# Furyton/Recommender-Baseline-Model

Hardware: AMD Instinct MI355X
Metric: training sequences/sec, SASRec L=200 d=128 at 1/2/4/8 MI355X; HR@10 parity (higher is better)
Workload: dtype bf16; 1 GPU; SASRec ML-1M shape (|items|=3416, seq_len=200, d=128, 2 blocks, 1 head, dropout 0.2); model=SASRec, global_batch=128, per_gpu_batch=128, seq_len=200, hidden=128, blocks=2, heads=1, num_items=3416, parallelism=dp1, hip_graph=True, bench_config=cfg2, sampler=host, steps_per_graph=10, full=False

## Files before the change

include/recsys_hip.h:

```cpp
#ifndef RECSYS_HIP_H
#define RECSYS_HIP_H
#include <stdint.h>
#ifdef __cplusplus
extern "C" {
#endif

#define RS_ERR_ARG 1001
#define RS_ERR_UNSUPPORTED 1002

typedef struct rs_epilogue {
  const float* bias;
  float alpha;
  int act;
  const void* aux;
  void* aux_out;
  int64_t ldaux;
  float drop_p;
  uint64_t drop_seed;
  const uint64_t* seed_base;
  int64_t drop_ld;
  const void* resid;
  int64_t ldres;
  const int64_t* rowmask_ids;
  int accumulate;
// ... 183 lines not shown
                          const float* divisor, void* f, float* pl, float* nl, float* dpl, float* dnl, void* dx,
                          float* lnpart, float* part, void* stream);

int64_t rs_touched_rows_ws_numel(int64_t rows);
int rs_touched_rows(const int64_t* ids, int64_t n, int64_t rows, int32_t* flags, int32_t* index, int32_t* count,
                    int32_t* ws, void* stream);
int rs_rows_pack(const float* src, int64_t rows, int64_t d, const int32_t* index, const int32_t* count,
                 float* compact, int64_t cap, void* stream);
int rs_rows_unpack(float* dst, int64_t rows, int64_t d, const int32_t* index, const float* compact, void* stream);

int64_t rs_sas_block_parts(int64_t M);
int rs_sas_block_out_bwd(int64_t M, int64_t d, const void* dxn, const int64_t* ids, const void* h1, const void* x1,
                         const float* mean2, const float* rstd2, const float* ln_w, const void* W2T, const void* W1T,
                         const void* WoT, void* dy2, void* da1, void* dx1, void* dout, float* part, float drop_p,
                         uint64_t salt1, uint64_t salt2, const uint64_t* seed_base, void* stream);
int rs_sas_block_out_bwd_delta(int64_t M, int64_t d, const void* dxn, const int64_t* ids, const void* h1,
                               const void* x1, const float* mean2, const float* rstd2, const float* ln_w,
                               const void* W2T, const void* W1T, const void* WoT, void* dy2, void* da1, void* dx1,
                               void* dout, float* part, float drop_p, uint64_t salt1, uint64_t salt2,
                               const uint64_t* seed_base, const void* o, float* delta, void* stream);
int rs_sas_block_in_bwd(int64_t M, int64_t d, const void* dq, const void* dkv, const void* dx1, const void* x,
                        const float* mean1, const float* rstd1, const float* ln_w, const void* WinT, void* dx,
                        float* part, void* stream);
int rs_transpose_bf16(int64_t nmat, const int64_t* desc, int64_t max_tiles, const void* src, void* dst,
                      void* stream);

typedef struct {
  const void* dY; int64_t lddy;
  const void* X;  int64_t ldx;
  int64_t N, K;
  float* dW;
  float* db;
} rs_wgrad_problem;
typedef struct {
  const float* src; int64_t stride; int64_t splits; int64_t n; float* out;
} rs_reduce_segment;
int64_t rs_wgrad_grouped_slab_numel(int nprob, const rs_wgrad_problem* probs, int64_t M, int64_t rows_per_split);
int rs_wgrad_grouped_tile(int nprob, const rs_wgrad_problem* probs);
int rs_wgrad_grouped_tile_max(int nprob, const rs_wgrad_problem* probs, int max_tile);
int rs_wgrad_grouped(int nprob, const rs_wgrad_problem* probs, int64_t M, int64_t rows_per_split, float* slab,
                     int64_t slab_numel, int nextra, const rs_reduce_segment* extra, void* stream);
int rs_wgrad_grouped_max(int nprob, const rs_wgrad_problem* probs, int64_t M, int64_t rows_per_split, float* slab,
                         int64_t slab_numel, int nextra, const rs_reduce_segment* extra, int max_tile, void* stream);

int rs_wgrad_grouped_pos(int nprob, const rs_wgrad_problem* probs, int64_t M, int64_t rows_per_split, float* slab,
                         int64_t slab_numel, int nextra, const rs_reduce_segment* extra, const int64_t* ids,
// ... 75 lines not shown
```

recommender-baseline-model_amd/_lib.py:

```python
import ctypes as C
import os

import torch

PKG = os.path.dirname(os.path.abspath(__file__))
LIB_PATH = os.path.join(PKG, "librecsys_hip.so" if not os.environ.get("RS_LIB_VARIANT")
                        else f"librecsys_hip.{os.environ['RS_LIB_VARIANT']}.so")

F32, BF16 = 0, 1

i32, i64, u64, f32, f64, vp = C.c_int, C.c_int64, C.c_uint64, C.c_float, C.c_double, C.c_void_p


class Epilogue(C.Structure):
    _fields_ = [
        ("bias", vp), ("alpha", f32), ("act", i32),
        ("aux", vp), ("aux_out", vp), ("ldaux", i64),
        ("drop_p", f32), ("drop_seed", u64), ("seed_base", vp), ("drop_ld", i64),
        ("resid", vp), ("ldres", i64),
        ("rowmask_ids", vp), ("accumulate", i32),
        ("post_drop_p", f32), ("post_drop_seed", u64), ("rows_dev", vp),
    ]


# ... 59 lines not shown
    "rs_vocab_shard_lse": [i64, i64, i64, vp, i64, vp, i64, vp, vp, vp, vp, vp],
    "rs_vocab_shard_label_logits": [i64, i64, vp, i64, vp, i64, vp, vp, i64, i64, vp, vp],
    "rs_vocab_shard_combine": [i32, i64, vp, vp, vp, vp, vp, vp],
    "rs_seed_advance": [vp, vp],
    "rs_sas_block_parts": [i64],
    "rs_touched_rows_ws_numel": [i64],
    "rs_touched_rows": [vp, i64, i64, vp, vp, vp, vp, vp],
    "rs_rows_pack": [vp, i64, i64, vp, vp, vp, i64, vp],
    "rs_rows_unpack": [vp, i64, i64, vp, vp, vp],
    "rs_sas_block_in": [i64, i64, vp, i64, vp, vp, f32, vp, vp, vp, vp, vp, vp, vp, vp, vp, vp],
    "rs_sas_block_in_count_parts": [i64],
    "rs_sas_block_grid": [i64],
    "rs_sas_block_out_head": [i64, i64, vp, vp, vp, vp, vp, vp, vp, f32, vp, vp, vp, vp, vp, vp, vp, vp, vp, vp, f32,
                              u64, u64, vp, vp, vp, vp, vp, vp, vp, i64, vp, vp, vp, vp, vp, vp, vp, vp, vp, vp],
    "rs_sas_block_in_embed": [i64, i64, vp, i64, vp, vp, f32, f32, u64, vp, vp, vp, vp, vp, vp, f32, vp, vp, vp, vp,
                              vp, vp, vp, vp, vp, vp],
    "rs_sas_block_out": [i64, i64, vp, vp, vp, vp, vp, vp, vp, f32, vp, vp, vp, vp, vp, vp, vp, vp, vp, vp, f32,
                         u64, u64, vp, vp],
    "rs_sas_block_out_bwd": [i64, i64, vp, vp, vp, vp, vp, vp, vp, vp, vp, vp, vp, vp, vp, vp, vp, f32, u64, u64,
                             vp, vp],
    "rs_sas_block_out_bwd_delta": [i64, i64, vp, vp, vp, vp, vp, vp, vp, vp, vp, vp, vp, vp, vp, vp, vp, f32, u64,
                                   u64, vp, vp, vp, vp],
    "rs_sas_block_in_bwd": [i64, i64, vp, vp, vp, vp, vp, vp, vp, vp, vp, vp, vp],
    "rs_wgrad_grouped": [i32, C.POINTER(WgradProblem), i64, i64, vp, i64, i32, C.POINTER(ReduceSegment), vp],
    "rs_reduce_segments": [i32, C.POINTER(ReduceSegment), i32, vp],
    "rs_wgrad_grouped_slab_numel": [i32, C.POINTER(WgradProblem), i64, i64],
    "rs_wgrad_grouped_tile": [i32, C.POINTER(WgradProblem)],
    "rs_wgrad_grouped_tile_max": [i32, C.POINTER(WgradProblem), i32],
    "rs_wgrad_grouped_max": [i32, C.POINTER(WgradProblem), i64, i64, vp, i64, i32, C.POINTER(ReduceSegment), i32, vp],
    "rs_item_index_ws_bytes": [i32, i64, i64, i64],
    "rs_item_index_build": [i32, vp, vp, vp, i64, i64, i64, vp, i64, vp],
    "rs_item_index_layout": [i32, i64, i64, i64, C.POINTER(i64)],
    "rs_sas_head_fwd": [i64, i64, vp, vp, vp, f32, vp, vp, vp, vp, vp, vp, vp, vp, vp, vp],
    "rs_sas_head_finish": [i64, vp, vp, vp, vp],
    "rs_sas_head_bwd": [i64, i64, vp, vp, vp, vp, vp, vp, vp, vp, vp, vp, vp, vp, vp, vp, vp, vp, vp, vp, vp],
    "rs_item_grad": [vp, i32, i64, i64, i64, vp, f32, f32, u64, vp, vp, vp, vp, vp, vp],
    "rs_item_grad_marked": [vp, i32, i64, i64, i64, vp, f32, f32, u64, vp, vp, vp, vp, vp, vp, vp, vp],
    "rs_item_grad_f32": [vp, i32, i64, i64, i64, vp, f32, f32, u64, vp, vp, vp, vp, vp, vp],
    "rs_wgrad_grouped_pos": [i32, C.POINTER(WgradProblem), i64, i64, vp, i64, i32, C.POINTER(ReduceSegment),
                             vp, i64, vp, i64, f32, u64, vp, vp, vp],
    "rs_wgrad_grouped_pos_stats": [i32, C.POINTER(WgradProblem), i64, i64, vp, i64, i32, C.POINTER(ReduceSegment),
                                   vp, i64, vp, i64, f32, u64, vp, vp, vp, i64, vp, vp, vp, vp],
    "rs_transpose_bf16": [i64, vp, i64, vp, vp, vp],
    "rs_sas_sample": [vp, vp, i64, i64, i64, i64, vp, u64, vp, vp, vp, vp],
    "rs_bert_mask": [vp, vp, i64, i64, i64, i64, f64, vp, vp, u64, vp, vp, vp],
    "rs_sas_sample_draws": [vp, vp, i64, i64, i64, i64, vp, u64, vp, vp, vp, vp, vp],
# ... 57 lines not shown
```

recommender-baseline-model_amd/csrc/rowchain.hip:

```cpp
#include "common.h"
#include "../../include/recsys_hip.h"

namespace rc {

#ifdef RC_PROF
__device__ unsigned long long g_rc_prof[4096 * 8 * 16];
#define RCPROF(slot)                                                                                 \
  do {                                                                                               \
    if ((threadIdx.x & 63) == 0) g_rc_prof[(blockIdx.x * 8 + (threadIdx.x >> 6)) * 16 + (slot)] = wall_clock64(); \
  } while (0)
#else
#define RCPROF(slot) \
  do {               \
  } while (0)
#endif

#ifndef RC_HEAD_PREFETCH
#define RC_HEAD_PREFETCH 1
#endif

#ifndef RC_NOSTORE
#define RC_NOSTORE 0
#endif

// ... 135 lines not shown
  float* rw = red + wave * 2 * D;
  float sg = 0.f, sgu = 0.f;
#pragma unroll
  for (int j = 0; j < Lay<D>::J; ++j) {
    const f32x4 w = vec4<D>(gw, j, g);
#pragma unroll
    for (int e = 0; e < 4; ++e) {
      const float gy = valid ? dy.v[j][e] : 0.f;
      const float u = (float)xr.v[j >> 1][4 * (j & 1) + e] - mu;
      const float gq = gy * w[e];
      const float pg = row16_sum(gy * (u * a)), pb = row16_sum(gy);
      if (cl == 0) {
        rw[feat(j, g, e)] += pg;
        rw[D + feat(j, g, e)] += pb;
      }
      sg += gq;
      sgu += gq * u;
      dy.v[j][e] = gq;
    }
  }
  sg = row_sum(sg);
  sgu = row_sum(sgu);
  const float mg = sg / (float)D, coef = a * a * a * sgu / (float)D;
#pragma unroll
  for (int j = 0; j < Lay<D>::J; ++j)
#pragma unroll
    for (int e = 0; e < 4; ++e)
      dy.v[j][e] = a * (dy.v[j][e] - mg) - coef * ((float)xr.v[j >> 1][4 * (j & 1) + e] - mu);
}

__device__ __forceinline__ void ln_zero(float* red, int D, int lane, int wave) {
  for (int i = lane; i < 2 * D; i += 64) red[wave * 2 * D + i] = 0.f;
}
template <int D>
__device__ __forceinline__ void ln_partials(const float* red, float* part, int tid) {
  __syncthreads();
  if (tid < 2 * D) {
    const int which = tid / D, c = tid % D;
    float s = 0.f;
#pragma unroll
    for (int w = 0; w < NW; ++w) s += red[(w * 2 + which) * D + c];
    part[((int64_t)blockIdx.x * 2 + which) * D + c] = s;
  }
}

__device__ __forceinline__ int64_t n_tiles(int64_t M) { return (M + TR - 1) / TR; }
// ... 104 lines not shown
  ln_fwd<D>(acc, lv + D, lv + 2 * D, o.eps, g, mu, rs);
  round_act<D>(acc, zr);
  if (!RC_NOSTORE) store_raw<D>(o.z, D, T.m, T.ok, zr, g);
  if (T.ok && g == 0) {
    o.mean[T.m] = mu;
    o.rstd[T.m] = rs;
  }
  zero<D>(acc);
  mm<D>(w1, zr, acc, lane);
  const bool drop = o.drop_p > 0.f;
#pragma unroll
  for (int j = 0; j < Lay<D>::J; ++j) {
    float dm[4] = {1.f, 1.f, 1.f, 1.f};
    if (drop) drop4(o.drop_p, o.s1, T.m, D, j, g, dm);
    const f32x4 bb = vec4<D>(lv + 3 * D, j, g);
#pragma unroll
    for (int e = 0; e < 4; ++e) acc.v[j][e] = fmaxf(acc.v[j][e] + bb[e], 0.f) * dm[e];
  }
  round_act<D>(acc, hr);
  if (!RC_NOSTORE) store_raw<D>(o.h1, D, T.m, T.ok, hr, g);
}
template <int D>
__device__ __forceinline__ void fwd_out_b(const Raw<D>& hr, const Raw<D>& zr, const Tile& T, const bf16* w2,
                                          const float* lv, const OutFwd& o, Raw<D>& xr, int lane) {
  const int g = lane >> 4;
  const bool keep = T.ok && o.ids[T.mc] != 0;
  Act<D> acc;
  zero<D>(acc);
  mm<D>(w2, hr, acc, lane);
  const bool drop = o.drop_p > 0.f;
#pragma unroll
  for (int j = 0; j < Lay<D>::J; ++j) {
    float dm[4] = {1.f, 1.f, 1.f, 1.f};
    if (drop) drop4(o.drop_p, o.s2, T.m, D, j, g, dm);
    const f32x4 bb = vec4<D>(lv + 4 * D, j, g);
#pragma unroll
    for (int e = 0; e < 4; ++e) {
      const float v = __builtin_fmaf(acc.v[j][e] + bb[e], dm[e], (float)zr.v[j >> 1][4 * (j & 1) + e]);
      acc.v[j][e] = keep ? v : 0.f;
    }
  }
  round_act<D>(acc, xr);
  store_raw<D>(o.xn, D, T.m, T.ok, xr, g);
}

template <int D>
__device__ __forceinline__ void bwd_in_a(const Raw<D>& kr, const Raw<D>& vr, const bf16* wk, const bf16* wv,
                                         Raw<D>& dxkv, int lane) {
  Act<D> acc;
  zero<D>(acc);
  mm<D>(wk, kr, acc, lane);
  mm<D>(wv, vr, acc, lane);
  round_act<D>(acc, dxkv);
}
template <int D>
__device__ __forceinline__ void bwd_in_b(const Raw<D>& qr, const Raw<D>& rr, const Raw<D>& xr, const Raw<D>& dxkv,
                                         const Tile& T, float mu, float rs, const bf16* wq, const float* lnw,
                                         float* red, Raw<D>& dxr, int lane, int wave) {
  const int g = lane >> 4;
  Act<D> dQ;
  Raw<D> r;
  to_act<D>(dQ, rr);
  mm<D>(wq, qr, dQ, lane);
  round_act<D>(dQ, r);
  ln_bwd<D>(dQ, xr, T.ok, lnw, mu, rs, red, lane, wave);
#pragma unroll
  for (int j = 0; j < Lay<D>::J; ++j)
#pragma unroll
    for (int e = 0; e < 4; ++e) dQ.v[j][e] += (float)dxkv.v[j >> 1][4 * (j & 1) + e];
  round_act<D>(dQ, dxr);
}

struct OutBwd {
  bf16 *dy2, *da1, *dx1, *dout;
  float* delta;
  const int64_t* ids;
  float drop_p;
  uint32_t s1, s2;
};
template <int D>
__device__ __forceinline__ void bwd_out_a(const Raw<D>& dr, const Raw<D>& hr, const Tile& T, const bf16* w2,
                                          const OutBwd& o, Raw<D>& dzr, Raw<D>& dar, int lane) {
  const int g = lane >> 4;
  const bool keep = T.ok && o.ids[T.mc] != 0;
  const bool drop = o.drop_p > 0.f;
  Act<D> acc;
  Raw<D> r;
#pragma unroll
  for (int j = 0; j < Lay<D>::J; ++j) {
    float dm[4] = {1.f, 1.f, 1.f, 1.f};
    if (drop) drop4(o.drop_p, o.s2, T.m, D, j, g, dm);
#pragma unroll
    for (int e = 0; e < 4; ++e) {
      const bf16 v = keep ? dr.v[j >> 1][4 * (j & 1) + e] : (bf16)0.f;
      dzr.v[j >> 1][4 * (j & 1) + e] = v;
      acc.v[j][e] = (float)v * dm[e];
    }
  }
  round_act<D>(acc, r);
  store_raw<D>(o.dy2, D, T.m, T.ok, r, g);
  zero<D>(acc);
  mm<D>(w2, r, acc, lane);
#pragma unroll
  for (int j = 0; j < Lay<D>::J; ++j) {
    float dm[4] = {1.f, 1.f, 1.f, 1.f};
    if (drop) drop4(o.drop_p, o.s1, T.m, D, j, g, dm);
#pragma unroll
    for (int e = 0; e < 4; ++e) acc.v[j][e] = ((float)hr.v[j >> 1][4 * (j & 1) + e] > 0.f ? acc.v[j][e] : 0.f) * dm[e];
  }
  round_act<D>(acc, dar);
  store_raw<D>(o.da1, D, T.m, T.ok, dar, g);
}
template <int D>
__device__ __forceinline__ void bwd_out_b(const Raw<D>& dar, const Raw<D>& xr, const Raw<D>& dzr, const Raw<D>& orr,
                                          const Tile& T, float mu, float rs, const bf16* w1, const bf16* wo,
                                          const float* lnw, const OutBwd& o, float* red, int lane, int wave) {
  const int g = lane >> 4;
  Raw<D> r;
  Act<D> dz;
  to_act<D>(dz, dzr);
  mm<D>(w1, dar, dz, lane);
  round_act<D>(dz, r);
  ln_bwd<D>(dz, xr, T.ok, lnw, mu, rs, red, lane, wave);
  round_act<D>(dz, r);
  store_raw<D>(o.dx1, D, T.m, T.ok, r, g);
  Act<D> acc;
  zero<D>(acc);
  mm<D>(wo, r, acc, lane);
  round_act<D>(acc, r);
  store_raw<D>(o.dout, D, T.m, T.ok, r, g);
  if (o.delta) {
    float dl = 0.f;
#pragma unroll
    for (int s = 0; s < Lay<D>::S; ++s)
// ... 367 lines not shown
  };
  if (t < tr.end) load_tile(tile_of(t, a.M, cl).mc);
  {
    const bf16* const W[3] = {a.WinT + D, a.WinT + 2 * D, a.WinT};
    const int64_t ldw[3] = {a.ldwt, a.ldwt, a.ldwt};
    stage_w<D, 3>(smem, W, ldw, wave, lane);
    const float* const V[1] = {a.ln_w};
    stage_v<D, 1>(reinterpret_cast<float*>(smem + L::W), V, tid);
  }
  ln_zero(red, D, lane, wave);
  __syncthreads();
  for (; t < tr.end; t += tr.step) {
    asm volatile("" ::: "memory");
    const Tile T = tile_of(t, a.M, cl);
    if (t != tr.first) load_tile(T.mc);
    Raw<D> dxkv, dxr;
    bwd_in_a<D>(kr, vr, wslot(smem, 0, WB), wslot(smem, 1, WB), dxkv, lane);
    bwd_in_b<D>(qr, rr, xr, dxkv, T, mu, rs, wslot(smem, 2, WB), lv, red, dxr, lane, wave);
    store_raw<D>(a.dx, D, T.m, T.ok, dxr, g);
  }
  ln_partials<D>(red, a.part, tid);
}

static int g_ncu = 0;
static int64_t grid_for(int64_t M) {
  if (g_ncu == 0) {
    int dev = 0, n = 0;
    if (hipGetDevice(&dev) == hipSuccess && hipDeviceGetAttribute(&n, hipDeviceAttributeMultiprocessorCount, dev) ==
                                                 hipSuccess && n > 0)
      g_ncu = n;
    else
      g_ncu = 256;
  }
  const int64_t nt = (M + TR - 1) / TR;
  return nt < g_ncu ? nt : g_ncu;
}
template <int D> static size_t lds_fwd() { return Smem<D, 3, 5, 0>::BYTES; }
template <int D, bool HEAD> static size_t lds_out() {
  return HEAD ? Smem<D, 3, 7, 1>::BYTES : Smem<D, 3, 5, 0>::BYTES;
}
template <int D> static size_t lds_bwd() { return Smem<D, 3, 1, 1>::BYTES; }

template <typename K>
static void set_lds(K kern, size_t bytes) {
  (void)hipFuncSetAttribute(reinterpret_cast<const void*>(kern), hipFuncAttributeMaxDynamicSharedMemorySize, (int)bytes);
}
template <int D, bool HEAD>
static void launch_out_t(const OutArgs& a, hipStream_t s) {
  constexpr auto k = block_out_kernel<D, HEAD>;
  const size_t lds = lds_out<D, HEAD>();
  set_lds(k, lds);
  hipLaunchKernelGGL(k, dim3((unsigned)grid_for(a.M)), dim3(NT), lds, s, a);
}
static int launch_out(const OutArgs& a, int64_t d, void* stream) {
  hipStream_t s = (hipStream_t)stream;
  const bool head = a.h.E != nullptr;
  if (d == 64) head ? launch_out_t<64, true>(a, s) : launch_out_t<64, false>(a, s);
  else if (d == 128) head ? launch_out_t<128, true>(a, s) : launch_out_t<128, false>(a, s);
  else return RS_ERR_UNSUPPORTED;
  return (int)hipGetLastError();
}

__global__ __launch_bounds__(256) void transpose_bf16_kernel(const int64_t* __restrict__ desc, const __bf16* src,
                                                             __bf16* dst) {
  __shared__ __bf16 t[64][66];
  const int64_t* dsc = desc + 6 * blockIdx.y;
  const int64_t rows = dsc[0], cols = dsc[1];
  const int64_t tc = cdiv(cols, 64);
  const int64_t tr = blockIdx.x / tc, tcc = blockIdx.x % tc;
  if (tr * 64 >= rows) return;
  const __bf16* sp = src + dsc[2];
  __bf16* dp = dst + dsc[4];
  const int64_t lds = dsc[3], ldd = dsc[5];
  for (int e = threadIdx.x; e < 64 * 64; e += 256) {
    const int r = e / 64, c = e % 64;
    const int64_t gr = tr * 64 + r, gc = tcc * 64 + c;
    t[r][c] = (gr < rows && gc < cols) ? sp[gr * lds + gc] : (__bf16)0.f;
  }
  __syncthreads();
  for (int e = threadIdx.x; e < 64 * 64; e += 256) {
    const int c = e / 64, r = e % 64;
    const int64_t gr = tr * 64 + r, gc = tcc * 64 + c;
    if (gr < rows && gc < cols) dp[gc * ldd + gr] = t[r][c];
// ... 119 lines not shown
  return (int)hipGetLastError();
}

int rs_sas_block_in_bwd(int64_t M, int64_t d, const void* dq, const void* dkv, const void* dx1, const void* x,
                        const float* mean1, const float* rstd1, const float* ln_w, const void* WinT, void* dx,
                        float* part, void* stream) {
  if (M <= 0) return RS_ERR_ARG;
  rc::InBwdArgs a = {M, (const __bf16*)dq, (const __bf16*)dkv, (const __bf16*)dx1, (const __bf16*)x, mean1, rstd1,
                     ln_w, (const __bf16*)WinT, 3 * d, (__bf16*)dx, part};
  const dim3 grid((unsigned)rc::grid_for(M));
  hipStream_t s = (hipStream_t)stream;
  if (d == 64) {
    rc::set_lds(rc::block_in_bwd_kernel<64>, rc::lds_bwd<64>());
    hipLaunchKernelGGL(rc::block_in_bwd_kernel<64>, grid, dim3(rc::NT), rc::lds_bwd<64>(), s, a);
  } else if (d == 128) {
    rc::set_lds(rc::block_in_bwd_kernel<128>, rc::lds_bwd<128>());
    hipLaunchKernelGGL(rc::block_in_bwd_kernel<128>, grid, dim3(rc::NT), rc::lds_bwd<128>(), s, a);
  } else {
    return RS_ERR_UNSUPPORTED;
  }
  return (int)hipGetLastError();
}

int rs_transpose_bf16(int64_t nmat, const int64_t* desc, int64_t max_tiles, const void* src, void* dst,
                      void* stream) {
  if (nmat <= 0 || max_tiles <= 0) return RS_ERR_ARG;
  hipLaunchKernelGGL(rc::transpose_bf16_kernel, dim3((unsigned)max_tiles, (unsigned)nmat), dim3(256), 0,
                     (hipStream_t)stream, desc, (const __bf16*)src, (__bf16*)dst);
  return (int)hipGetLastError();
}

}
```

recommender-baseline-model_amd/models/sas_model/sas.py:

```python
import math
import os

import torch
import torch.nn as nn

from ... import ops
from ...engine_util import Workspace, as_ids, capture_event, compute_dtype, require_cuda, site_salt
from ...flat import FlatParams

LN_EPS = 1e-8
SAS_LOSSES = ("bce", "ce")


class PointWiseFeedForward(nn.Module):

    def __init__(self, hidden_units, dropout_rate):
        super().__init__()
        self.conv1 = nn.Conv1d(hidden_units, hidden_units, kernel_size=1)
        self.conv2 = nn.Conv1d(hidden_units, hidden_units, kernel_size=1)
        self.dropout_rate = dropout_rate


class SAS(nn.Module):
    def __init__(self, args):
# ... 124 lines not shown
        grads = [eng.flat.view(n, grad) for n in eng.flat.names]
        return (None, None, None, None, *grads)


class SASEngine:

    def __init__(self, model: SAS, flat: FlatParams):
        self.m = model
        self.flat = flat
        self.d = model.hidden
        self.L = model.num_blocks
        self.H = model.heads
        self.Dh = self.d // self.H
        self.p = float(model.dropout_rate)
        self.dt = model.cdtype
        self.dev = flat.device
        if self.dt == torch.bfloat16:
            flat.enable_bf16()
        self.ws = Workspace(self.dev)
        self.seed_base = torch.zeros(1, dtype=torch.int64, device=self.dev)
        self.external_seed = False
        self.adam_transposes = False
        self._wT = None
        salt0 = int(torch.randint(0, 2 ** 62, (1,)).item())
        self.salt = {"emb": site_salt(salt0, 0)}
        for i in range(self.L):
            self.salt[f"attn{i}"] = site_salt(salt0, 1 + 4 * i)
            self.salt[f"ffn1_{i}"] = site_salt(salt0, 2 + 4 * i)
            self.salt[f"ffn2_{i}"] = site_salt(salt0, 3 + 4 * i)

    def sync_compute_weights(self):
        f = self.flat
        if f.bf16 is not None:
            if not f.stale:
                ops.cast_bf16(f.data, f.bf16)
            else:
                a = 0
                for lo, hi in sorted(f.stale) + [(f.numel, f.numel)]:
                    if lo > a:
                        ops.cast_bf16(f.data[a:lo], f.bf16[a:lo])
                    a = max(a, hi)
            if self._wT is not None:
                self._refresh_transposed()

    def transposed_spec(self):
        if not self.adam_transposes or self._wT is None:
# ... 125 lines not shown
            return (self.Wf(f"attention_layernorms.{i}.weight"), self.Wf(f"attention_layernorms.{i}.bias"),
                    b["Q"], b["mu1"], b["r1"], Win[:d], bin_[:d], b["q"], Win[d:], bin_[d:], b["kv"])

        def out_args(i):
            pre, fw, b = f"attention_layers.{i}.", f"forward_layers.{i}.", lay[i]
            return (b["o"], b["Q"], self.W(pre + "out_proj.weight"), self.Wf(pre + "out_proj.bias"), b["x1"],
                    self.Wf(f"forward_layernorms.{i}.weight"), self.Wf(f"forward_layernorms.{i}.bias"), LN_EPS,
                    b["z"], b["mu2"], b["r2"], self.W(fw + "conv1.weight"), self.Wf(fw + "conv1.bias"), b["h1"],
                    self.W(fw + "conv2.weight"), self.Wf(fw + "conv2.bias"), b["xn"], ids, p,
                    self.salt[f"ffn1_{i}"], self.salt[f"ffn2_{i}"], sb)

        ln_w, ln_b, Q, mu1, r1, Wq, bq, q, Wkv, bkv, kv = in_args(0)
        if emb is not None:
            ops.sas_block_in_embed(*emb, ln_w, ln_b, LN_EPS, Q, mu1, r1, Wq, bq, q, Wkv, bkv, kv)
        else:
            ops.sas_block_in(x, ln_w, ln_b, LN_EPS, Q, mu1, r1, Wq, bq, q, Wkv, bkv, kv)
        if after_first is not None:
            after_first()
        xs = [x]
        for i in range(L):
            b = lay[i]
            ops.attn_fwd(B, T, H, Dh, b["q"], b["kv"][:, :d], b["kv"][:, d:], b["o"], b["lse"], 1.0 / math.sqrt(Dh),
                         0, ids, p, self.salt[f"attn{i}"], sb)
            if head is not None and i == L - 1:
                ops.sas_block_out_head(out_args(i), *head)
            else:
                ops.sas_block_out(*out_args(i))
            if i + 1 < L:
                ln_w, ln_b, Q, mu1, r1, Wq, bq, q, Wkv, bkv, kv = in_args(i + 1)
                ops.sas_block_in(b["xn"], ln_w, ln_b, LN_EPS, Q, mu1, r1, Wq, bq, q, Wkv, bkv, kv)
            xs.append(b["xn"])
        for i in range(L):
            b = lay[i]
            for k_ in ("Q", "mu1", "r1", "q", "kv", "o", "lse", "x1", "z", "mu2", "r2", "h1"):
                s[k_].append(b[k_])
            s["x"].append(xs[i])
        return xs[L]

    @property
    def fused_head(self):
        return ops.sas_block_fused_ok(self.d, self.dt)

    def backward(self, s, dpl, dnl, grad, loss_out=None, divisor=None, split=None, aux_out=None):
        B, T, p, ids = s["B"], s["T"], s["p"], s["ids"]
        M, d, H, Dh, L = B * T, self.d, self.H, self.Dh, self.L
        sb = s["sb"]
        e = self._buf
        G = lambda n: self.flat.view(n, grad)
        slab = self.ws.get("slab", (ops.wgrad_slab_numel(M, 2 * d, d),), torch.float32)
        wln = self.ws.get("ln", (2 * 512 * d,), torch.float32)
        wat = self.ws.get("attn", (B * H * T,), torch.float32)

        fused = ops.sas_block_fused_ok(d, self.dt)
# ... 265 lines not shown
        wat = self.ws.get("attn", (B * H * T,), torch.float32)
        probs, segs = [], list(extra_segs)
        g = [dict(dy2=e("dy2", (M, d)), da1=e("da1", (M, d)), dx1=e("dx1", (M, d)), do=e("do", (M, d)),
                  dq=e("dq", (M, d)), dkv=e("dkv", (M, 2 * d))) for _ in range(L)]

        dl = [self.ws.get(f"attn_delta{i}", (B * H * T,), torch.float32) for i in range(L)] if H == 1 else None

        def out_bwd_args(i):
            return (ids, s["h1"][i], s["x1"][i], s["mu2"][i], s["r2"][i], self.Wf(f"forward_layernorms.{i}.weight"),
                    wT[i, 5], wT[i, 4], wT[i, 3], g[i]["dy2"], g[i]["da1"], g[i]["dx1"], g[i]["do"], lnp[i, 0], p,
                    self.salt[f"ffn1_{i}"], self.salt[f"ffn2_{i}"], sb, s["o"][i] if dl else None, dl[i] if dl else None)

        def in_bwd_args(i):
            return (g[i]["dq"], g[i]["dkv"], g[i]["dx1"], s["x"][i], s["mu1"][i], s["r1"][i],
                    self.Wf(f"attention_layernorms.{i}.weight"), wT[i, 0:3].reshape(d, 3 * d))

        ops.sas_block_out_bwd(dx, *out_bwd_args(L - 1))
        for i in reversed(range(L)):
            pre, fw = f"attention_layers.{i}.", f"forward_layers.{i}."
            dq, dkv, kv = g[i]["dq"], g[i]["dkv"], s["kv"][i]
            ops.attn_bwd(B, T, H, Dh, s["q"][i], kv[:, :d], kv[:, d:], s["o"][i], g[i]["do"], s["lse"][i], dq,
                         dkv[:, :d], dkv[:, d:], 1.0 / math.sqrt(Dh), 0, ids, p, self.salt[f"attn{i}"], sb,
                         dl[i] if dl else wat, delta_in=bool(dl))
            dxi = e("dxi", (M, d))
            ops.sas_block_in_bwd(*in_bwd_args(i), dxi, lnp[i, 1])
            if i > 0:
                ops.sas_block_out_bwd(dxi, *out_bwd_args(i - 1))
            dx = dxi
            Gin, Gb = G(pre + "in_proj_weight"), G(pre + "in_proj_bias")
            probs += [(g[i]["dy2"], s["h1"][i], G(fw + "conv2.weight"), G(fw + "conv2.bias")),
                      (g[i]["da1"], s["z"][i], G(fw + "conv1.weight"), G(fw + "conv1.bias")),
                      (g[i]["dx1"], s["o"][i], G(pre + "out_proj.weight"), G(pre + "out_proj.bias")),
                      (dq, s["Q"][i], Gin[:d], Gb[:d]),
                      (dkv, s["x"][i], Gin[d:], Gb[d:])]
            segs += ops.ln_partial_segments(lnp[i, 0], M, d, G(f"forward_layernorms.{i}.weight"),
                                            G(f"forward_layernorms.{i}.bias"))
            segs += ops.ln_partial_segments(lnp[i, 1], M, d, G(f"attention_layernorms.{i}.weight"),
                                            G(f"attention_layernorms.{i}.bias"))
        rows = self._wgrad_rows(M, 6 * L)
        wslab = self.ws.get("wslab", (ops.wgrad_grouped_slab_numel([(d, d)] * 4 * L + [(2 * d, d)] * L, M, rows),),
                            torch.float32)
        join, fork = None, None
        if tail is not None:
            fork = capture_event()
            fork.record(torch.cuda.current_stream())
        ops.wgrad_grouped(probs, M, rows, wslab, extra=segs, pos=pos(dx) if pos is not None else None)
        if tail is not None:
            self._side.wait_event(fork)
            with torch.cuda.stream(self._side):
                tail(dx)
# ... 30 lines not shown
```

recommender-baseline-model_amd/ops.py:

```python
import ctypes as C
import os

import torch

from . import _lib
from ._lib import BF16, F32, Epilogue, call, ptr, stream

ACT_NONE, ACT_RELU, ACT_GELU, ACT_RELU_BWD, ACT_GELU_BWD = (
    _lib.ACT_NONE, _lib.ACT_RELU, _lib.ACT_GELU, _lib.ACT_RELU_BWD, _lib.ACT_GELU_BWD)


STAMP_KINDS = {1: "attn_bwd", 2: "wgrad_grouped", 3: "vocab_ce_fwd"}


def kernel_stamps(buf, step, kinds=()):
    mask = sum(1 << k for k, n in STAMP_KINDS.items() if n in kinds)
    call("rs_kernel_stamps", ptr(buf), ptr(step), mask)


def read_kernel_stamps(buf, khz):
    import numpy as np
    h = buf.cpu().numpy().view(np.uint64)
    steps, marks, W = int(h[1]), int(h[2]), int(h[3])
    rec = h[4:4 + steps * marks * (1 + W)].reshape(steps, marks, 1 + W)
# ... 471 lines not shown

def sas_block_out(o, Q, Wo, bo, x1, ln_w, ln_b, eps, z, mean, rstd, W1, b1, h1, W2, b2, xn, ids, drop_p,
                  salt1, salt2, seed_base):
    M, d = o.shape
    call("rs_sas_block_out", M, d, ptr(o), ptr(Q), ptr(Wo), ptr(bo), ptr(x1), ptr(ln_w), ptr(ln_b), eps, ptr(z),
         ptr(mean), ptr(rstd), ptr(W1), ptr(b1), ptr(h1), ptr(W2), ptr(b2), ptr(xn), ptr(ids), drop_p, salt1,
         salt2, ptr(seed_base), stream())


def sas_block_out_bwd(dxn, ids, h1, x1, mean2, rstd2, ln_w, W2T, W1T, WoT, dy2, da1, dx1, dout, part, drop_p, salt1,
                      salt2, seed_base, o=None, delta=None):
    M, d = dxn.shape
    call("rs_sas_block_out_bwd_delta", M, d, ptr(dxn), ptr(ids), ptr(h1), ptr(x1), ptr(mean2), ptr(rstd2),
         ptr(ln_w), ptr(W2T), ptr(W1T), ptr(WoT), ptr(dy2), ptr(da1), ptr(dx1), ptr(dout), ptr(part), drop_p, salt1,
         salt2, ptr(seed_base), ptr(o), ptr(delta), stream())


def sas_block_in_bwd(dq, dkv, dx1, x, mean1, rstd1, ln_w, WinT, dx, part):
    M, d = dq.shape
    call("rs_sas_block_in_bwd", M, d, ptr(dq), ptr(dkv), ptr(dx1), ptr(x), ptr(mean1), ptr(rstd1), ptr(ln_w),
         ptr(WinT), ptr(dx), ptr(part), stream())


def touched_rows_ws_numel(rows):
    return int(_lib.lib().rs_touched_rows_ws_numel(rows))


def touched_rows(ids, rows, flags, index, count, ws):
    call("rs_touched_rows", ptr(ids), ids.numel(), rows, ptr(flags), ptr(index), ptr(count), ptr(ws), stream())


def rows_pack(src, index, count, compact):
    rows, d = src.shape
    call("rs_rows_pack", ptr(src), rows, d, ptr(index), ptr(count), ptr(compact), compact.shape[0], stream())


def rows_unpack(dst, index, compact):
    rows, d = dst.shape
    call("rs_rows_unpack", ptr(dst), rows, d, ptr(index), ptr(compact), stream())


def sas_block_parts(M):
    return int(_lib.lib().rs_sas_block_parts(M))


def ln_partial_segments(part, M, d, dgamma, dbeta, nb=None):
# ... 242 lines not shown
```

Measured before the change: 463,700 sequences/s.

## Fuse SASRec block boundary: out-proj/FFN with next block's in-proj, fwd and bwd

Adds kernels that join one block's output stage (out-proj, LN, FFN) with the next block's input stage (LN, Q and KV projections) in the forward pass, and the matching input-backward with the previous block's output-backward in the backward pass. Intermediate rows stay in registers across the boundary and weights are staged into LDS slots, so the xn/dxi round-trip through global memory and one launch per boundary go away. For d=128 the six weight slots do not all fit, so the kernel restages two slots mid-kernel behind extra barriers. It is on by default through an env flag and falls back to the two separate kernels when the grid cannot give every tile its own wave.

```diff
diff --git a/include/recsys_hip.h b/include/recsys_hip.h
--- a/include/recsys_hip.h
+++ b/include/recsys_hip.h
@@ -229,6 +229,20 @@
 int rs_sas_block_in_bwd(int64_t M, int64_t d, const void* dq, const void* dkv, const void* dx1, const void* x,
                         const float* mean1, const float* rstd1, const float* ln_w, const void* WinT, void* dx,
                         float* part, void* stream);
+int rs_sas_block_boundary_fused(int64_t M, int64_t d);
+int rs_sas_block_out_in(int64_t M, int64_t d, const void* o, const void* Q, const void* Wo, const float* bo, void* x1,
+                        const float* ln_w, const float* ln_b, float eps, void* z, float* mean, float* rstd,
+                        const void* W1, const float* b1, void* h1, const void* W2, const float* b2, void* xn,
+                        const int64_t* ids, float drop_p, uint64_t salt1, uint64_t salt2, const uint64_t* seed_base,
+                        const float* ln1_w, const float* ln1_b, float eps1, void* Qn, float* mean1, float* rstd1,
+                        const void* Wq, const float* bq, void* q, const void* Wkv, const float* bkv, void* kv,
+                        void* stream);
+int rs_sas_block_in_out_bwd(int64_t M, int64_t d, const void* dq, const void* dkv, const void* dx1, const void* x,
+                            const float* mean1, const float* rstd1, const float* ln1_w, const void* WinT, void* dx,
+                            float* part1, const int64_t* ids, const void* h1, const void* x1, const float* mean2,
+                            const float* rstd2, const float* ln2_w, const void* W2T, const void* W1T, const void* WoT,
+                            void* dy2, void* da1, void* dx1o, void* dout, float* part2, float drop_p, uint64_t salt1,
+                            uint64_t salt2, const uint64_t* seed_base, const void* o, float* delta, void* stream);
 int rs_transpose_bf16(int64_t nmat, const int64_t* desc, int64_t max_tiles, const void* src, void* dst,
                       void* stream);
 
diff --git a/recommender-baseline-model_amd/_lib.py b/recommender-baseline-model_amd/_lib.py
--- a/recommender-baseline-model_amd/_lib.py
+++ b/recommender-baseline-model_amd/_lib.py
@@ -105,6 +105,11 @@
     "rs_sas_block_out_bwd_delta": [i64, i64, vp, vp, vp, vp, vp, vp, vp, vp, vp, vp, vp, vp, vp, vp, vp, f32, u64,
                                    u64, vp, vp, vp, vp],
     "rs_sas_block_in_bwd": [i64, i64, vp, vp, vp, vp, vp, vp, vp, vp, vp, vp, vp],
+    "rs_sas_block_boundary_fused": [i64, i64],
+    "rs_sas_block_out_in": [i64, i64, vp, vp, vp, vp, vp, vp, vp, f32, vp, vp, vp, vp, vp, vp, vp, vp, vp, vp, f32,
+                            u64, u64, vp, vp, vp, f32, vp, vp, vp, vp, vp, vp, vp, vp, vp, vp],
+    "rs_sas_block_in_out_bwd": [i64, i64, vp, vp, vp, vp, vp, vp, vp, vp, vp, vp, vp, vp, vp, vp, vp, vp, vp, vp, vp,
+                                vp, vp, vp, vp, vp, f32, u64, u64, vp, vp, vp, vp],
     "rs_wgrad_grouped": [i32, C.POINTER(WgradProblem), i64, i64, vp, i64, i32, C.POINTER(ReduceSegment), vp],
     "rs_reduce_segments": [i32, C.POINTER(ReduceSegment), i32, vp],
     "rs_wgrad_grouped_slab_numel": [i32, C.POINTER(WgradProblem), i64, i64],
diff --git a/recommender-baseline-model_amd/csrc/rowchain.hip b/recommender-baseline-model_amd/csrc/rowchain.hip
--- a/recommender-baseline-model_amd/csrc/rowchain.hip
+++ b/recommender-baseline-model_amd/csrc/rowchain.hip
@@ -181,6 +181,8 @@
   sg = row_sum(sg);
   sgu = row_sum(sgu);
   const float mg = sg / (float)D, coef = a * a * a * sgu / (float)D;
+#pragma unroll
+  for (int j = 0; j < Lay<D>::J; ++j) asm volatile("" : "+v"(dy.v[j]));
 #pragma unroll
   for (int j = 0; j < Lay<D>::J; ++j)
 #pragma unroll
@@ -331,9 +333,8 @@
 }
 template <int D>
 __device__ __forceinline__ void fwd_out_b(const Raw<D>& hr, const Raw<D>& zr, const Tile& T, const bf16* w2,
-                                          const float* lv, const OutFwd& o, Raw<D>& xr, int lane) {
+                                          const float* lv, const OutFwd& o, Raw<D>& xr, int lane, bool keep) {
   const int g = lane >> 4;
-  const bool keep = T.ok && o.ids[T.mc] != 0;
   Act<D> acc;
   zero<D>(acc);
   mm<D>(w2, hr, acc, lane);
@@ -351,6 +352,11 @@
   }
   round_act<D>(acc, xr);
   store_raw<D>(o.xn, D, T.m, T.ok, xr, g);
+}
+template <int D>
+__device__ __forceinline__ void fwd_out_b(const Raw<D>& hr, const Raw<D>& zr, const Tile& T, const bf16* w2,
+                                          const float* lv, const OutFwd& o, Raw<D>& xr, int lane) {
+  fwd_out_b<D>(hr, zr, T, w2, lv, o, xr, lane, T.ok && o.ids[T.mc] != 0);
 }
 
 template <int D>
@@ -389,9 +395,8 @@
 };
 template <int D>
 __device__ __forceinline__ void bwd_out_a(const Raw<D>& dr, const Raw<D>& hr, const Tile& T, const bf16* w2,
-                                          const OutBwd& o, Raw<D>& dzr, Raw<D>& dar, int lane) {
+                                          const OutBwd& o, Raw<D>& dzr, Raw<D>& dar, int lane, bool keep) {
   const int g = lane >> 4;
-  const bool keep = T.ok && o.ids[T.mc] != 0;
   const bool drop = o.drop_p > 0.f;
   Act<D> acc;
   Raw<D> r;
@@ -419,6 +424,11 @@
   }
   round_act<D>(acc, dar);
   store_raw<D>(o.da1, D, T.m, T.ok, dar, g);
+}
+template <int D>
+__device__ __forceinline__ void bwd_out_a(const Raw<D>& dr, const Raw<D>& hr, const Tile& T, const bf16* w2,
+                                          const OutBwd& o, Raw<D>& dzr, Raw<D>& dar, int lane) {
+  bwd_out_a<D>(dr, hr, T, w2, o, dzr, dar, lane, T.ok && o.ids[T.mc] != 0);
 }
 template <int D>
 __device__ __forceinline__ void bwd_out_b(const Raw<D>& dar, const Raw<D>& xr, const Raw<D>& dzr, const Raw<D>& orr,
@@ -832,6 +842,155 @@
   ln_partials<D>(red, a.part, tid);
 }
 
+template <int D> struct Roll {
+  static constexpr bool ON = 6 * Lay<D>::WBYTES > 128 * 1024;
+  static constexpr int WB = Lay<D>::WBYTES, XB = ON ? 16 : Lay<D>::WBYTES;
+};
+template <int D>
+__device__ __forceinline__ void stage_slot(char* slot, const bf16* W, int64_t ldw, int wave, int lane) {
+  const bf16* const Wm[1] = {W};
+  const int64_t ld[1] = {ldw};
+  stage_w<D, 1>(slot, Wm, ld, wave, lane);
+}
+__device__ __forceinline__ const bf16* wimg(const char* slot) { return reinterpret_cast<const bf16*>(slot); }
+typedef __attribute__((ext_vector_type(4))) uint32_t u32x4;
+template <int D>
+__device__ __forceinline__ void as_loaded(Raw<D>& r) {
+#pragma unroll
+  for (int s = 0; s < Lay<D>::S; ++s) {
+    u32x4 t = __builtin_bit_cast(u32x4, r.v[s]);
+    asm volatile("" : "+v"(t));
+    r.v[s] = __builtin_bit_cast(bf16x8, t);
+  }
+}
+#define RC_BOUNDARY_SLOTS(D)                                                                            \
+  __shared__ __attribute__((aligned(16))) char w0[Roll<D>::WB], w1[Roll<D>::WB], w2[Roll<D>::WB], w3[Roll<D>::WB], \
+      w4[Roll<D>::XB], w5[Roll<D>::XB]
+
+template <int D>
+__global__ __launch_bounds__(NT) void block_out_in_kernel(OutArgs a, InArgs b) {
+  typedef Roll<D> R;
+  RC_BOUNDARY_SLOTS(D);
+  __shared__ __attribute__((aligned(16))) float lv[10 * D];
+  const int tid = threadIdx.x, lane = tid & 63, wave = __builtin_amdgcn_readfirstlane(tid >> 6), g = lane >> 4,
+            cl = lane & 15;
+  const TileRange tr = tiles_of_wave(n_tiles(a.M), wave);
+  const bool has = tr.first < tr.end;
+  const Tile T = tile_of(has ? tr.first : 0, a.M, cl);
+  const OutFwd of = out_fwd_of(a);
+  Raw<D> orr, Qr;
+  int64_t id = 0;
+  if (has) {
+    load_raw<D>(orr, a.o, D, T.mc, g);
+    load_raw<D>(Qr, a.Q, D, T.mc, g);
+    id = a.ids[T.mc];
+  }
+  const bf16* const Wk = b.Wkv;
+  const bf16* const Wv = b.Wkv + (int64_t)D * D;
+  stage_slot<D>(w0, a.Wo, D, wave, lane);
+  stage_slot<D>(w1, a.W1, D, wave, lane);
+  stage_slot<D>(w2, a.W2, D, wave, lane);
+  stage_slot<D>(w3, b.Wq, D, wave, lane);
+  if constexpr (!R::ON) {
+    stage_slot<D>(w4, Wk, D, wave, lane);
+    stage_slot<D>(w5, Wv, D, wave, lane);
+  }
+  {
+    const float* const V[10] = {a.bo, a.ln_w, a.ln_b, a.b1, a.b2, b.ln_w, b.ln_b, b.bq, b.bkv, b.bkv + D};
+    stage_v<D, 10>(lv, V, tid);
+  }
+  __syncthreads();
+  asm volatile("" : "+v"(id));
+  Raw<D> zr, hr, xr;
+  if (has) fwd_out_a<D>(orr, Qr, T, wimg(w0), wimg(w1), lv, of, zr, hr, lane);
+  if constexpr (R::ON) {
+    __syncthreads();
+    stage_slot<D>(w0, Wk, D, wave, lane);
+    stage_slot<D>(w1, Wv, D, wave, lane);
+  }
+  asm volatile("" ::: "memory");
+  if (has) {
+    fwd_out_b<D>(hr, zr, T, wimg(w2), lv, of, xr, lane, T.ok && id != 0);
+    asm volatile("" ::: "memory");
+    as_loaded<D>(xr);
+    fwd_in_q<D>(xr, T, wimg(w3), lv + 5 * D, b.eps, b.Q, b.mean, b.rstd, b.q, lane);
+  }
+  if constexpr (R::ON) __syncthreads();
+  asm volatile("" ::: "memory");
+  if (has) fwd_in_kv<D>(xr, T, wimg(R::ON ? w0 : w4), wimg(R::ON ? w1 : w5), lv + 5 * D, b.kv, lane);
+}
+
+template <int D>
+__global__ __launch_bounds__(NT) void block_in_out_bwd_kernel(InBwdArgs a, OutBwdArgs b) {
+  typedef Roll<D> R;
+  RC_BOUNDARY_SLOTS(D);
+  __shared__ __attribute__((aligned(16))) float lv[2 * D];
+  __shared__ __attribute__((aligned(16))) float red[NW * 2 * D], red2[NW * 2 * D];
+  const int tid = threadIdx.x, lane = tid & 63, wave = __builtin_amdgcn_readfirstlane(tid >> 6), g = lane >> 4,
+            cl = lane & 15;
+  const TileRange tr = tiles_of_wave(n_tiles(a.M), wave);
+  const bool has = tr.first < tr.end;
+  const Tile T = tile_of(has ? tr.first : 0, a.M, cl);
+  const OutBwd ob = out_bwd_of(b);
+  Raw<D> kr, vr, qr, rr, xr;
+  float mu = 0.f, rs = 0.f;
+  int64_t id = 0;
+  if (has) {
+    load_raw<D>(kr, a.dkv, 2 * D, T.mc, g);
+    load_raw<D>(vr, a.dkv + D, 2 * D, T.mc, g);
+    load_raw<D>(qr, a.dq, D, T.mc, g);
+    load_raw<D>(rr, a.dx1, D, T.mc, g);
+    load_raw<D>(xr, a.x, D, T.mc, g);
+    mu = a.mean1[T.mc];
+    rs = a.rstd1[T.mc];
+    id = b.ids[T.mc];
+  }
+  stage_slot<D>(w0, a.WinT + D, a.ldwt, wave, lane);
+  stage_slot<D>(w1, a.WinT + 2 * D, a.ldwt, wave, lane);
+  stage_slot<D>(w2, a.WinT, a.ldwt, wave, lane);
+  stage_slot<D>(w3, b.W2T, D, wave, lane);
+  if constexpr (!R::ON) {
+    stage_slot<D>(w4, b.W1T, D, wave, lane);
+    stage_slot<D>(w5, b.WoT, D, wave, lane);
+  }
+  {
+    const float* const V[2] = {a.ln_w, b.ln_w};
+    stage_v<D, 2>(lv, V, tid);
+  }
+  ln_zero(red, D, lane, wave);
+  ln_zero(red2, D, lane, wave);
+  __syncthreads();
+  asm volatile("" : "+v"(id));
+  Raw<D> dxkv, dxr, hr, x1r, orr, dzr, dar;
+  float mu2 = 0.f, rs2 = 0.f;
+  if (has) {
+    bwd_in_a<D>(kr, vr, wimg(w0), wimg(w1), dxkv, lane);
+    load_raw<D>(hr, b.h1, D, T.mc, g);
+    load_raw<D>(x1r, b.x1, D, T.mc, g);
+    if (b.delta) load_raw<D>(orr, b.o, D, T.mc, g);
+    mu2 = b.mean2[T.mc];
+    rs2 = b.rstd2[T.mc];
+    bwd_in_b<D>(qr, rr, xr, dxkv, T, mu, rs, wimg(w2), lv, red, dxr, lane, wave);
+  }
+  if constexpr (R::ON) {
+    __syncthreads();
+    stage_slot<D>(w0, b.W1T, D, wave, lane);
+    stage_slot<D>(w1, b.WoT, D, wave, lane);
+  }
+  asm volatile("" ::: "memory");
+  if (has) {
+    as_loaded<D>(dxr);
+    bwd_out_a<D>(dxr, hr, T, wimg(w3), ob, dzr, dar, lane, T.ok && id != 0);
+  }
+  if constexpr (R::ON) __syncthreads();
+  asm volatile("" ::: "memory");
+  if (has)
+    bwd_out_b<D>(dar, x1r, dzr, orr, T, mu2, rs2, wimg(R::ON ? w0 : w4), wimg(R::ON ? w1 : w5), lv + D, ob, red2,
+                 lane, wave);
+  ln_partials<D>(red, a.part, tid);
+  ln_partials<D>(red2, b.part, tid);
+}
+
 static int g_ncu = 0;
 static int64_t grid_for(int64_t M) {
   if (g_ncu == 0) {
@@ -869,6 +1028,18 @@
   else if (d == 128) head ? launch_out_t<128, true>(a, s) : launch_out_t<128, false>(a, s);
   else return RS_ERR_UNSUPPORTED;
   return (int)hipGetLastError();
+}
+
+static bool boundary_fused(int64_t M, int64_t d) {
+  return M > 0 && (d == 64 || d == 128) && (M + TR - 1) / TR <= grid_for(M) * NW;
+}
+template <int D>
+static void launch_out_in_t(const OutArgs& a, const InArgs& b, hipStream_t s) {
+  hipLaunchKernelGGL(block_out_in_kernel<D>, dim3((unsigned)grid_for(a.M)), dim3(NT), 0, s, a, b);
+}
+template <int D>
+static void launch_in_out_bwd_t(const InBwdArgs& a, const OutBwdArgs& b, hipStream_t s) {
+  hipLaunchKernelGGL(block_in_out_bwd_kernel<D>, dim3((unsigned)grid_for(a.M)), dim3(NT), 0, s, a, b);
 }
 
 __global__ __launch_bounds__(256) void transpose_bf16_kernel(const int64_t* __restrict__ desc, const __bf16* src,
@@ -1034,6 +1205,60 @@
   return (int)hipGetLastError();
 }
 
+int rs_sas_block_boundary_fused(int64_t M, int64_t d) { return rc::boundary_fused(M, d) ? 1 : 0; }
+
+int rs_sas_block_out_in(int64_t M, int64_t d, const void* o, const void* Q, const void* Wo, const float* bo, void* x1,
+                        const float* ln_w, const float* ln_b, float eps, void* z, float* mean, float* rstd,
+                        const void* W1, const float* b1, void* h1, const void* W2, const float* b2, void* xn,
+                        const int64_t* ids, float drop_p, uint64_t salt1, uint64_t salt2, const uint64_t* seed_base,
+                        const float* ln1_w, const float* ln1_b, float eps1, void* Qn, float* mean1, float* rstd1,
+                        const void* Wq, const float* bq, void* q, const void* Wkv, const float* bkv, void* kv,
+                        void* stream) {
+  if (M <= 0) return RS_ERR_ARG;
+  if (d != 64 && d != 128) return RS_ERR_UNSUPPORTED;
+  if (!rc::boundary_fused(M, d)) {
+    const int rc1 = rs_sas_block_out(M, d, o, Q, Wo, bo, x1, ln_w, ln_b, eps, z, mean, rstd, W1, b1, h1, W2, b2, xn,
+                                     ids, drop_p, salt1, salt2, seed_base, stream);
+    if (rc1) return rc1;
+    return rs_sas_block_in(M, d, xn, d, ln1_w, ln1_b, eps1, Qn, mean1, rstd1, Wq, bq, q, Wkv, bkv, kv, stream);
+  }
+  rc::OutArgs a = {M, (const __bf16*)o, (const __bf16*)Q, (const __bf16*)Wo, bo, (__bf16*)x1, ln_w, ln_b, eps,
+                   (__bf16*)z, mean, rstd, (const __bf16*)W1, b1, (__bf16*)h1, (const __bf16*)W2, b2, (__bf16*)xn,
+                   ids, drop_p, salt1, salt2, seed_base};
+  rc::InArgs b = {M, (const __bf16*)xn, d, ln1_w, ln1_b, eps1, (__bf16*)Qn, mean1, rstd1, (const __bf16*)Wq, bq,
+                  (__bf16*)q, (const __bf16*)Wkv, bkv, (__bf16*)kv};
+  hipStream_t s = (hipStream_t)stream;
+  if (d == 64) rc::launch_out_in_t<64>(a, b, s);
+  else rc::launch_out_in_t<128>(a, b, s);
+  return (int)hipGetLastError();
+}
+
+int rs_sas_block_in_out_bwd(int64_t M, int64_t d, const void* dq, const void* dkv, const void* dx1, const void* x,
+                            const float* mean1, const float* rstd1, const float* ln1_w, const void* WinT, void* dx,
+                            float* part1, const int64_t* ids, const void* h1, const void* x1p, const float* mean2,
+                            const float* rstd2, const float* ln2_w, const void* W2T, const void* W1T, const void* WoT,
+                            void* dy2, void* da1, void* dx1p, void* dout, float* part2, float drop_p, uint64_t salt1,
+                            uint64_t salt2, const uint64_t* seed_base, const void* o, float* delta, void* stream) {
+  if (M <= 0 || !o != !delta) return RS_ERR_ARG;
+  if (d != 64 && d != 128) return RS_ERR_UNSUPPORTED;
+  if (!rc::boundary_fused(M, d)) {
+    if (!dx) return RS_ERR_ARG;
+    const int rc1 = rs_sas_block_in_bwd(M, d, dq, dkv, dx1, x, mean1, rstd1, ln1_w, WinT, dx, part1, stream);
+    if (rc1) return rc1;
+    return rs_sas_block_out_bwd_delta(M, d, dx, ids, h1, x1p, mean2, rstd2, ln2_w, W2T, W1T, WoT, dy2, da1, dx1p, dout,
+                                      part2, drop_p, salt1, salt2, seed_base, o, delta, stream);
+  }
+  rc::InBwdArgs a = {M, (const __bf16*)dq, (const __bf16*)dkv, (const __bf16*)dx1, (const __bf16*)x, mean1, rstd1,
+                     ln1_w, (const __bf16*)WinT, 3 * d, nullptr, part1};
+  rc::OutBwdArgs b = {M, nullptr, ids, (const __bf16*)h1, (const __bf16*)x1p, mean2, rstd2, ln2_w,
+                      (const __bf16*)W2T, (const __bf16*)W1T, (const __bf16*)WoT, (__bf16*)dy2, (__bf16*)da1,
+                      (__bf16*)dx1p, (__bf16*)dout, part2, drop_p, salt1, salt2, seed_base, (const __bf16*)o, delta};
+  hipStream_t s = (hipStream_t)stream;
+  if (d == 64) rc::launch_in_out_bwd_t<64>(a, b, s);
+  else rc::launch_in_out_bwd_t<128>(a, b, s);
+  return (int)hipGetLastError();
+}
+
 int rs_transpose_bf16(int64_t nmat, const int64_t* desc, int64_t max_tiles, const void* src, void* dst,
                       void* stream) {
   if (nmat <= 0 || max_tiles <= 0) return RS_ERR_ARG;
diff --git a/recommender-baseline-model_amd/models/sas_model/sas.py b/recommender-baseline-model_amd/models/sas_model/sas.py
--- a/recommender-baseline-model_amd/models/sas_model/sas.py
+++ b/recommender-baseline-model_amd/models/sas_model/sas.py
@@ -170,6 +170,7 @@
         self.external_seed = False
         self.adam_transposes = False
         self._wT = None
+        self.boundary_fuse = os.environ.get("RS_SAS_BOUNDARY_FUSE", "1") != "0"
         salt0 = int(torch.randint(0, 2 ** 62, (1,)).item())
         self.salt = {"emb": site_salt(salt0, 0)}
         for i in range(self.L):
@@ -341,13 +342,17 @@
             b = lay[i]
             ops.attn_fwd(B, T, H, Dh, b["q"], b["kv"][:, :d], b["kv"][:, d:], b["o"], b["lse"], 1.0 / math.sqrt(Dh),
                          0, ids, p, self.salt[f"attn{i}"], sb)
-            if head is not None and i == L - 1:
+            if i + 1 < L:
+                ln_w, ln_b, Q, mu1, r1, Wq, bq, q, Wkv, bkv, kv = in_args(i + 1)
+                if self.boundary_fuse:
+                    ops.sas_block_out_in(out_args(i), ln_w, ln_b, LN_EPS, Q, mu1, r1, Wq, bq, q, Wkv, bkv, kv)
+                else:
+                    ops.sas_block_out(*out_args(i))
+                    ops.sas_block_in(b["xn"], ln_w, ln_b, LN_EPS, Q, mu1, r1, Wq, bq, q, Wkv, bkv, kv)
+            elif head is not None:
                 ops.sas_block_out_head(out_args(i), *head)
             else:
                 ops.sas_block_out(*out_args(i))
-            if i + 1 < L:
-                ln_w, ln_b, Q, mu1, r1, Wq, bq, q, Wkv, bkv, kv = in_args(i + 1)
-                ops.sas_block_in(b["xn"], ln_w, ln_b, LN_EPS, Q, mu1, r1, Wq, bq, q, Wkv, bkv, kv)
             xs.append(b["xn"])
         for i in range(L):
             b = lay[i]
@@ -659,10 +664,14 @@
             ops.attn_bwd(B, T, H, Dh, s["q"][i], kv[:, :d], kv[:, d:], s["o"][i], g[i]["do"], s["lse"][i], dq,
                          dkv[:, :d], dkv[:, d:], 1.0 / math.sqrt(Dh), 0, ids, p, self.salt[f"attn{i}"], sb,
                          dl[i] if dl else wat, delta_in=bool(dl))
-            dxi = e("dxi", (M, d))
-            ops.sas_block_in_bwd(*in_bwd_args(i), dxi, lnp[i, 1])
-            if i > 0:
-                ops.sas_block_out_bwd(dxi, *out_bwd_args(i - 1))
+            if i > 0 and self.boundary_fuse:
+                dxi = None if ops.sas_block_boundary_fused(M, d) else e("dxi", (M, d))
+                ops.sas_block_in_out_bwd(in_bwd_args(i), dxi, lnp[i, 1], out_bwd_args(i - 1))
+            else:
+                dxi = e("dxi", (M, d))
+                ops.sas_block_in_bwd(*in_bwd_args(i), dxi, lnp[i, 1])
+                if i > 0:
+                    ops.sas_block_out_bwd(dxi, *out_bwd_args(i - 1))
             dx = dxi
             Gin, Gb = G(pre + "in_proj_weight"), G(pre + "in_proj_bias")
             probs += [(g[i]["dy2"], s["h1"][i], G(fw + "conv2.weight"), G(fw + "conv2.bias")),
diff --git a/recommender-baseline-model_amd/ops.py b/recommender-baseline-model_amd/ops.py
--- a/recommender-baseline-model_amd/ops.py
+++ b/recommender-baseline-model_amd/ops.py
@@ -517,6 +517,31 @@
          ptr(WinT), ptr(dx), ptr(part), stream())
 
 
+def sas_block_boundary_fused(M, d):
+    return bool(_lib.lib().rs_sas_block_boundary_fused(M, d))
+
+
+def sas_block_out_in(out_args, ln1_w, ln1_b, eps1, Qn, mean1, rstd1, Wq, bq, q, Wkv, bkv, kv):
+    (o, Q, Wo, bo, x1, ln_w, ln_b, eps, z, mean, rstd, W1, b1, h1, W2, b2, xn, ids, drop_p, salt1, salt2,
+     seed_base) = out_args
+    M, d = o.shape
+    call("rs_sas_block_out_in", M, d, ptr(o), ptr(Q), ptr(Wo), ptr(bo), ptr(x1), ptr(ln_w), ptr(ln_b), eps, ptr(z),
+         ptr(mean), ptr(rstd), ptr(W1), ptr(b1), ptr(h1), ptr(W2), ptr(b2), ptr(xn), ptr(ids), drop_p, salt1, salt2,
+         ptr(seed_base), ptr(ln1_w), ptr(ln1_b), eps1, ptr(Qn), ptr(mean1), ptr(rstd1), ptr(Wq), ptr(bq), ptr(q),
+         ptr(Wkv), ptr(bkv), ptr(kv), stream())
+
+
+def sas_block_in_out_bwd(in_args, dx, part1, out_args):
+    dq, dkv, dx1, x, mean1, rstd1, ln1_w, WinT = in_args
+    (ids, h1, x1, mean2, rstd2, ln2_w, W2T, W1T, WoT, dy2, da1, dx1o, dout, part2, drop_p, salt1, salt2,
+     seed_base, o, delta) = out_args
+    M, d = dq.shape
+    call("rs_sas_block_in_out_bwd", M, d, ptr(dq), ptr(dkv), ptr(dx1), ptr(x), ptr(mean1), ptr(rstd1), ptr(ln1_w),
+         ptr(WinT), ptr(dx), ptr(part1), ptr(ids), ptr(h1), ptr(x1), ptr(mean2), ptr(rstd2), ptr(ln2_w), ptr(W2T),
+         ptr(W1T), ptr(WoT), ptr(dy2), ptr(da1), ptr(dx1o), ptr(dout), ptr(part2), drop_p, salt1, salt2,
+         ptr(seed_base), ptr(o), ptr(delta), stream())
+
+
 def touched_rows_ws_numel(rows):
     return int(_lib.lib().rs_touched_rows_ws_numel(rows))
 
```

Measured after the change: 485,100 sequences/s (median of 6 runs). +4.6%, better.
